# imironhead/ml_super_resolution

Hardware: AMD Instinct MI355X
Metric: VDSR-20 training patches/sec (41x41, batch 256 per GPU); fwd HR megapixels/sec alongside (higher is better)
Workload: dtype f32; 1 GPU; BASELINE configs[2]: VDSR 20-layer 3x3x64 residual, RGB, batch 256x41x41 per GPU, fwd+bwd+TF-Adam, random-init weights; global_batch=256, patch=41, parallelism=dp1

## Files before the change

include/srx.h:

```cpp
#ifndef SRX_H_
#define SRX_H_

#include <stddef.h>
#include <stdint.h>

#ifdef __cplusplus
extern "C" {
#endif

typedef void* srx_stream_t;

typedef enum {
    SRX_OK = 0,
    SRX_ERR_BAD_ARG = -1,
    SRX_ERR_UNSUPPORTED = -2,
    SRX_ERR_WORKSPACE = -3,
    SRX_ERR_LAUNCH = -4,
    SRX_ERR_ALIGN = -5
} srx_status;

typedef enum { SRX_PAD_SAME = 0, SRX_PAD_VALID = 1 } srx_pad_mode;

typedef enum {
    SRX_ACT_NONE = 0,
    SRX_ACT_RELU = 1,
    SRX_ACT_TANH = 2,
    SRX_ACT_LRELU = 3,
    SRX_ACT_SIGMOID = 4
} srx_act;

typedef enum { SRX_OP_FWD = 0, SRX_OP_BWD_DATA = 1, SRX_OP_BWD_FILTER = 2 } srx_conv_op;

typedef enum { SRX_PRECISION_FP32 = 0, SRX_PRECISION_BF16X3 = 1 } srx_precision;

typedef struct {
    int32_t N, H, W, Cin, Cout, KH, KW;
    int32_t stride;
    int32_t pad_mode;
    int32_t act;
    int32_t post_add_relu;
    int32_t precision;
    int32_t subpixel_r;
} srx_conv_desc;

const char* srx_version(void);
const char* srx_last_error(void);

int srx_set_conv_path(int pipelined);

int srx_set_wgrad_path(int path);

int srx_conv_chain(const srx_conv_desc* d, int op, int in_act, int layers, const float* const* x, const float* const* w,
                   const float* const* bias, const float* const* aux, float* const* y, srx_stream_t stream);

int srx_conv_chain_supported(const srx_conv_desc* d, int op, int in_act);

int srx_set_chain(int on);

int srx_conv2d_precision_supported(const srx_conv_desc* d, int op);

size_t srx_conv2d_workspace_bytes(const srx_conv_desc* d, int op);

int srx_conv2d_fwd(const srx_conv_desc* d, const float* x, const float* w, const float* bias,
                   const float* skip, float* y, void* ws, size_t ws_bytes, srx_stream_t stream);

int srx_conv2d_bwd_data(const srx_conv_desc* d, const float* dpre, const float* w,
                        const float* x_in, int in_act, float* dx_out, void* ws, size_t ws_bytes,
                        srx_stream_t stream);

int srx_conv2d_bwd_data_acc(const srx_conv_desc* d, const float* dpre, const float* w, const float* dx_acc,
                            float* dx_out, void* ws, size_t ws_bytes, srx_stream_t stream);

int srx_conv2d_bwd_filter(const srx_conv_desc* d, const float* x, const float* dpre, float* dw,
                          float* dbias, const float* w_for_decay, float wd_scale, void* ws,
                          size_t ws_bytes, srx_stream_t stream);

int srx_conv2d_bwd_filter_partials(const srx_conv_desc* d, const float* x, const float* dpre, void* ws,
                                   size_t ws_bytes, int* n_partials, srx_stream_t stream);
int srx_conv2d_bwd_filter_reduce(const srx_conv_desc* d, const void* ws, int n_partials, float* dw,
                                 float* dbias, const float* w_for_decay, float wd_scale,
                                 srx_stream_t stream);

int srx_act_bwd(const float* dy, const float* y, float* dpre, size_t numel, int act,
                srx_stream_t stream);

int srx_depth_to_space(const float* in, float* out, int N, int H, int W, int C, int r,
                       srx_stream_t stream);

int srx_stream_copy(const void* in, void* out, size_t bytes, srx_stream_t stream);

// ... 145 lines not shown
```

ml_super_resolution_amd/_lib.py:

```python
import ctypes
import os

_HERE = os.path.dirname(os.path.abspath(__file__))
LIB_PATH = os.path.join(_HERE, 'libsrx.so')

SRX_OK = 0
PAD_SAME, PAD_VALID = 0, 1
ACT_NONE, ACT_RELU, ACT_TANH, ACT_LRELU, ACT_SIGMOID = 0, 1, 2, 3, 4
OP_FWD, OP_BWD_DATA, OP_BWD_FILTER = 0, 1, 2
PRECISION_FP32, PRECISION_BF16X3 = 0, 1
PRECISION_BY_NAME = {'highest': PRECISION_FP32, 'high': PRECISION_BF16X3}

ACT_BY_NAME = {None: ACT_NONE, 'none': ACT_NONE, 'relu': ACT_RELU, 'tanh': ACT_TANH,
               'lrelu': ACT_LRELU, 'leaky_relu': ACT_LRELU, 'sigmoid': ACT_SIGMOID}
PAD_BY_NAME = {'same': PAD_SAME, 'valid': PAD_VALID}

EXPORTS = [
    'srx_version', 'srx_last_error', 'srx_set_conv_path', 'srx_set_wgrad_path', 'srx_set_chain', 'srx_conv_chain', 'srx_conv_chain_supported', 'srx_conv2d_precision_supported', 'srx_conv2d_workspace_bytes', 'srx_conv2d_fwd',
    'srx_conv2d_bwd_data', 'srx_conv2d_bwd_filter', 'srx_conv2d_bwd_filter_partials', 'srx_conv2d_bwd_filter_reduce', 'srx_act_bwd', 'srx_depth_to_space',
    'srx_space_to_depth', 'srx_stream_copy', 'srx_mse_fwd_bwd', 'srx_l2_loss', 'srx_reduce_scratch_bytes',
    'srx_adam_tf_step', 'srx_adam_tf_step_dev', 'srx_momentum_clip_step', 'srx_rownorm_loss_fwd_bwd', 'srx_psnr', 'srx_ssim', 'srx_ssim_scratch_bytes', 'srx_saturate_u8', 'srx_affine', 'srx_u8_to_unit_float', 'srx_gaussian_blur', 'srx_resize_bilinear',
    'srx_upsample_nearest', 'srx_upsample_nearest_bwd', 'srx_add_relu_grad',
    'srx_conv2d_bwd_data_acc', 'srx_conv3x3_blocked', 'srx_conv3x3_blocked_bwd_filter_workspace_bytes', 'srx_conv3x3_blocked_bwd_filter',
    'srx_conv3x3_blocked_ex', 'srx_conv3x3_blocked_bwd_filter_ex_workspace_bytes', 'srx_conv3x3_blocked_bwd_filter_ex',
    'srx_espcn_forward', 'srx_espcn_forward_keep', 'srx_debug_poison_lds', 'srx_srcnn_forward', 'srx_maxpool2x2', 'srx_maxpool2x2_bwd', 'srx_maxpool2x2_bwd_masked', 'srx_subsample2', 'srx_subsample2_bwd',
    'srx_channel_blocks_to_nhwc', 'srx_nhwc_to_channel_blocks', 'srx_channel_normalize', 'srx_channel_normalize_bwd',
    'srx_extract_patches16', 'srx_texture_gram', 'srx_texture_gram_bwd', 'srx_pil_resample_ksize', 'srx_pil_resample_coeffs', 'srx_resample_u8', 'srx_u8_to_pm1', 'srx_log_loss', 'srx_vgg_preprocess', 'srx_add_scaled', 'srx_resize_bicubic_tf', 'srx_column_sums', 'srx_gemm_workspace_bytes', 'srx_gemm',
]


class SrxError(RuntimeError):
    pass


class ConvDesc(ctypes.Structure):
    _fields_ = [(n, ctypes.c_int32) for n in
                ('N', 'H', 'W', 'Cin', 'Cout', 'KH', 'KW', 'stride', 'pad_mode', 'act',
                 'post_add_relu', 'precision', 'subpixel_r')]


class GemmDesc(ctypes.Structure):
    _fields_ = ([(n, ctypes.c_int32) for n in ('M', 'N', 'K', 'batch')] +
                [(n, ctypes.c_int64) for n in ('a_row_stride', 'a_col_stride', 'a_batch_stride', 'b_row_stride',
                                               'b_col_stride', 'b_batch_stride', 'c_row_stride', 'c_col_stride',
                                               'c_batch_stride')] +
                [('alpha', ctypes.c_float), ('act', ctypes.c_int32), ('accumulate', ctypes.c_int32)])


_lib = None


def lib():
    global _lib
    if _lib is not None:
        return _lib
    if not os.path.exists(LIB_PATH):
        raise SrxError('libsrx.so not found at %s -- build it with `make -C %s` (or '
                       '__graft_entry__.build()); there is no CPU fallback' %
                       (LIB_PATH, os.path.join(_HERE, 'csrc')))
    import torch
    L = ctypes.CDLL(LIB_PATH)
    vp, sz, i, f = ctypes.c_void_p, ctypes.c_size_t, ctypes.c_int, ctypes.c_float
    dp = ctypes.POINTER(ConvDesc)
    L.srx_version.restype = ctypes.c_char_p
    L.srx_last_error.restype = ctypes.c_char_p
    L.srx_set_conv_path.argtypes = [i]
    L.srx_set_wgrad_path.argtypes = [i]
    L.srx_set_chain.argtypes = [i]
    L.srx_conv_chain_supported.argtypes = [dp, i, i]
    L.srx_conv_chain.argtypes = [dp, i, i, i, vp, vp, vp, vp, vp, vp]
    L.srx_conv2d_precision_supported.argtypes = [dp, i]
    L.srx_conv2d_workspace_bytes.argtypes = [dp, i]
    L.srx_conv2d_workspace_bytes.restype = sz
    L.srx_reduce_scratch_bytes.restype = sz
    L.srx_conv2d_fwd.argtypes = [dp, vp, vp, vp, vp, vp, vp, sz, vp]
    L.srx_conv2d_bwd_data.argtypes = [dp, vp, vp, vp, i, vp, vp, sz, vp]
    L.srx_conv2d_bwd_filter.argtypes = [dp, vp, vp, vp, vp, vp, f, vp, sz, vp]
    L.srx_conv2d_bwd_filter_partials.argtypes = [dp, vp, vp, vp, sz, ctypes.POINTER(ctypes.c_int), vp]
    L.srx_conv2d_bwd_filter_reduce.argtypes = [dp, vp, i, vp, vp, vp, f, vp]
    L.srx_act_bwd.argtypes = [vp, vp, vp, sz, i, vp]
    L.srx_depth_to_space.argtypes = [vp, vp, i, i, i, i, i, vp]
    L.srx_space_to_depth.argtypes = [vp, vp, i, i, i, i, i, vp]
    L.srx_stream_copy.argtypes = [vp, vp, sz, vp]
    L.srx_mse_fwd_bwd.argtypes = [vp, vp, sz, f, vp, i, vp, vp, vp]
    L.srx_l2_loss.argtypes = [vp, vp, sz, f, vp, i, vp, vp]
    L.srx_adam_tf_step.argtypes = [vp, vp, vp, vp, sz, f, f, f, f, ctypes.c_int64, f, vp]
    L.srx_adam_tf_step_dev.argtypes = [vp, vp, vp, vp, sz, vp, f, f, f, f, vp]
    L.srx_momentum_clip_step.argtypes = [vp, vp, vp, sz, f, f, f, f, vp]
    L.srx_rownorm_loss_fwd_bwd.argtypes = [vp, vp, sz, sz, vp, vp, vp, vp]
    L.srx_psnr.argtypes = [vp, vp, vp, i, sz, f, vp]
    L.srx_ssim.argtypes = [vp, vp, vp, i, i, i, i, f, vp, vp]
    L.srx_ssim_scratch_bytes.argtypes = [i]
    L.srx_ssim_scratch_bytes.restype = sz
    L.srx_saturate_u8.argtypes = [vp, vp, sz, vp]
    L.srx_affine.argtypes = [vp, vp, sz, f, f, vp]
    L.srx_u8_to_unit_float.argtypes = [vp, vp, sz, vp]
    L.srx_gaussian_blur.argtypes = [vp, vp, vp, i, i, i, i, f, vp]
    L.srx_resize_bilinear.argtypes = [vp, vp, i, i, i, i, i, i, vp]
    L.srx_upsample_nearest.argtypes = [vp, vp, i, i, i, i, i, vp]
    L.srx_upsample_nearest_bwd.argtypes = [vp, vp, i, i, i, i, i, vp]
    L.srx_add_relu_grad.argtypes = [vp, vp, vp, vp, sz, vp]
# ... 47 lines not shown
```

ml_super_resolution_amd/csrc/conv_narrow.hip:

```cpp
#include "launchers.h"
namespace srx {
typedef float f32x3 __attribute__((ext_vector_type(3)));
typedef unsigned u32x3v __attribute__((ext_vector_type(3)));

template <int CTRL>
__device__ __forceinline__ float dpp_add(float v) {
    const int moved = __builtin_amdgcn_update_dpp(0, __float_as_int(v), CTRL, 0xf, 0xf, false);
    return v + __int_as_float(moved);
}

struct PixWalk {
    int n, oh, ow;
    __device__ __forceinline__ void init(unsigned p, int OH, int OW) {
        const unsigned t = p / (unsigned)OW;
        ow = (int)(p - t * (unsigned)OW);
        n = (int)(t / (unsigned)OH);
        oh = (int)(t - (unsigned)n * (unsigned)OH);
    }
    __device__ __forceinline__ void step16(int OH, int OW) { step(16, OH, OW); }
    __device__ __forceinline__ void step(int d, int OH, int OW) {
        ow += d;
        while (ow >= OW) {
            ow -= OW;
            oh += 1;
            if (oh == OH) { oh = 0; n += 1; }
        }
    }
};
template <int KH, int KW>
__device__ __forceinline__ void tap_offsets(int (&off)[KH * KW], const PixWalk& q, bool live, int H, int W, int pad_t, int pad_l,
                                            int PB, int lane_b) {
    const int centre = ((q.n * H + q.oh - pad_t) * W + (q.ow - pad_l)) * PB + lane_b;
    bool rok[KH], cok[KW];
#pragma unroll
    for (int kh = 0; kh < KH; ++kh) rok[kh] = live && (unsigned)(q.oh + kh - pad_t) < (unsigned)H;
#pragma unroll
    for (int kw = 0; kw < KW; ++kw) cok[kw] = (unsigned)(q.ow + kw - pad_l) < (unsigned)W;
#pragma unroll
    for (int kh = 0; kh < KH; ++kh)
#pragma unroll
        for (int kw = 0; kw < KW; ++kw)
            off[kh * KW + kw] = (rok[kh] && cok[kw]) ? centre + (kh * W + kw) * PB : kOobOffset;
}

template <int KH, int KW, int CIN, int CO>
__global__ __launch_bounds__(256) void conv_narrow_kernel(const ConvArgs a, long total_px, int iters) {
    static_assert(CIN == 64, "16 lanes x 4 channels per pixel");
    constexpr int TAPS = KH * KW;
    const int c4 = threadIdx.x & 15;
    const int sub = threadIdx.x >> 4;
    float wr[TAPS][4][CO];
#pragma unroll
    for (int t = 0; t < TAPS; ++t)
#pragma unroll
        for (int e = 0; e < 4; ++e)
#pragma unroll
            for (int c = 0; c < CO; ++c) wr[t][e][c] = a.w[((size_t)t * CIN + 4 * c4 + e) * CO + c];
    float bias[CO];
#pragma unroll
    for (int c = 0; c < CO; ++c) bias[c] = a.bias ? a.bias[c] : 0.0f;
    const __amdgpu_buffer_rsrc_t xrs = __builtin_amdgcn_make_buffer_rsrc(const_cast<float*>(a.x), 0,
                                                                         a.N * a.H * a.W * CIN * 4, 0x00020000);
    const unsigned p0 = blockIdx.x * (unsigned)iters * 16u + sub;
    PixWalk q;
    q.init(p0 < (unsigned)total_px ? p0 : 0u, a.OH, a.OW);
    for (int it = 0; it < iters; ++it, q.step16(a.OH, a.OW)) {
        const unsigned p = p0 + (unsigned)it * 16u;
        const bool live = p < (unsigned)total_px;
        int off[TAPS];
        tap_offsets<KH, KW>(off, q, live, a.H, a.W, a.pad_t, a.pad_l, CIN * 4, 16 * c4);
        f32x4 v[TAPS];
#pragma unroll
        for (int tp = 0; tp < TAPS; ++tp)
            v[tp] = __builtin_bit_cast(f32x4, __builtin_amdgcn_raw_buffer_load_b128(xrs, off[tp], 0, 0));
        float acc[CO];
#pragma unroll
        for (int c = 0; c < CO; ++c) acc[c] = 0.0f;
// ... 155 lines not shown
```

ml_super_resolution_amd/csrc/launchers.h:

```cpp
#pragma once
#include "conv_kernels.hip.h"

namespace srx {

struct ConvKey {
    int kh, kw, cinp, nch;
    bool wt;
};

bool launch_conv_k3c64(const ConvKey& k, const ConvArgs& a, int grid, size_t lds, hipStream_t s, hipError_t* err);
bool launch_conv_k3c32(const ConvKey& k, const ConvArgs& a, int grid, size_t lds, hipStream_t s, hipError_t* err);
bool launch_conv_c4(const ConvKey& k, const ConvArgs& a, int grid, size_t lds, hipStream_t s, hipError_t* err);
bool launch_conv_misc(const ConvKey& k, const ConvArgs& a, int grid, size_t lds, hipStream_t s, hipError_t* err);
bool launch_pipe_k3c64(const ConvKey& k, const ConvArgs& a, int grid, size_t lds, hipStream_t s, hipError_t* err);
bool launch_pipe_other(const ConvKey& k, const ConvArgs& a, int grid, size_t lds, hipStream_t s, hipError_t* err);
bool launch_wgrad_narrow(const ConvKey& k, const WgradArgs& a, int grid, hipStream_t s, hipError_t* err);
bool launch_conv_narrow(const ConvKey& k, const ConvArgs& a, hipStream_t s, hipError_t* err);
bool launch_conv_1x1(const ConvKey& k, const ConvArgs& a, long min_pixels, hipStream_t s, hipError_t* err);
bool launch_conv_rows3x3(const ConvKey& k, const ConvArgs& a, long min_pixels, hipStream_t s, hipError_t* err);
bool launch_conv_pack3(const ConvKey& k, const ConvArgs& a, long min_pixels, hipStream_t s, hipError_t* err);
bool launch_conv_kwrows(const ConvKey& k, const ConvArgs& a, long min_pixels, hipStream_t s, hipError_t* err);
bool launch_pipe_strip(const ConvKey& k, const ConvArgs& a, int grid, size_t lds, hipStream_t s, hipError_t* err);
bool launch_conv_generic(const ConvKey& k, const ConvArgs& a, int grid, size_t lds, hipStream_t s, hipError_t* err);
bool launch_wgrad(const ConvKey& k, const WgradArgs& a, int grid, size_t lds, hipStream_t s, hipError_t* err);
bool launch_wgrad_generic(const ConvKey& k, const WgradArgs& a, int grid, size_t lds, hipStream_t s, hipError_t* err);
bool launch_wgrad_lin(const ConvKey& k, const WgradArgs& a, int grid, size_t lds, hipStream_t s, hipError_t* err);
bool launch_wgrad_lin_pack3(const ConvKey& k, const WgradArgs& a, int grid, size_t lds, hipStream_t s, hipError_t* err);
bool launch_wgrad_lin_strip(const ConvKey& k, const WgradArgs& a, int grid, size_t lds, hipStream_t s, hipError_t* err);
bool launch_wgrad_pipe(const ConvKey& k, const WgradArgs& a, int grid, size_t lds, hipStream_t s, hipError_t* err);
bool launch_wgrad_kwcols(const ConvKey& k, const WgradArgs& a, int max_partials, long min_pixels, int* n_partials, hipStream_t s, hipError_t* err);
bool launch_wgrad_1x1(const ConvKey& k, const WgradArgs& a, int max_partials, int* n_partials, hipStream_t s, hipError_t* err);
bool launch_wgrad_rows_full(const ConvKey& k, const WgradArgs& a, int grid, size_t lds, hipStream_t s, hipError_t* err);
bool launch_wgrad_rows_strip(const ConvKey& k, const WgradArgs& a, int grid, size_t lds, hipStream_t s, hipError_t* err);
bool launch_wgrad_lin_pairs(const ConvKey& k, const WgradPairs& q, int grid, int pairs, bool strips, size_t lds, hipStream_t s, hipError_t* err);

__attribute__((weak)) hipError_t launch_conv_chain(bool wt, bool aux, const ConvArgs& a, const ChainPtrs& c, int grid, size_t lds, hipStream_t s);

hipError_t launch_reduce_partials(const float* part, int G, int stride, int wn, int cout, float* dw, float* dbias,
                                  const float* w, float wd, hipStream_t s);
hipError_t launch_reduce_partials_pairs(const float* part, int G, int stride, int wn, int cout, float* dw, float* dbias,
                                        int pairs, int cob, hipStream_t s);

template <typename K, typename A>
inline hipError_t launch_with_lds(K kernel, const A& a, int grid, size_t lds, hipStream_t s, int grid_y = 1) {
    static thread_local const void* configured[64];
    static thread_local int n_configured = 0;
    const void* fn = reinterpret_cast<const void*>(kernel);
    bool known = false;
    for (int i = 0; i < n_configured; ++i) known |= (configured[i] == fn);
    if (!known) {
        hipError_t e = hipFuncSetAttribute(fn, hipFuncAttributeMaxDynamicSharedMemorySize, 160 * 1024);
        if (e != hipSuccess) return e;
        if (n_configured < 64) configured[n_configured++] = fn;
    }
    hipLaunchKernelGGL(kernel, dim3(grid, grid_y), dim3(256), lds, s, a);
    return hipGetLastError();
}

template <typename K>
inline hipError_t launch_chain_with_lds(K kernel, const ConvArgs& a, const ChainPtrs& c, int grid, size_t lds, hipStream_t s) {
    static thread_local const void* configured[8];
    static thread_local int n_configured = 0;
    const void* fn = reinterpret_cast<const void*>(kernel);
    bool known = false;
    for (int i = 0; i < n_configured; ++i) known |= (configured[i] == fn);
    if (!known) {
        hipError_t e = hipFuncSetAttribute(fn, hipFuncAttributeMaxDynamicSharedMemorySize, 160 * 1024);
        if (e != hipSuccess) return e;
        if (n_configured < 8) configured[n_configured++] = fn;
// ... 80 lines not shown
```

ml_super_resolution_amd/csrc/srx_api.hip:

```cpp
#include <math.h>
#include <stdarg.h>
#include <atomic>
#include <stdio.h>
#include <stdlib.h>
#include <string.h>

#include "../../include/srx.h"
#include "elementwise.h"
#include "launchers.h"
#include "bf16x3.h"

using namespace srx;

namespace {

thread_local char g_err[512] = "";

struct Knobs {
    int pipe_default, narrow, wgrad_lin, wgrad_pipe, wgrad_pipe_strip, wgrad_rows_full, wgrad_1x1, wgrad_pack3, kwrows_min_pixels, big_route_min_pixels, strip_d2s, conv_1x1_min_pixels, pack3_dgrad;
    int chain;
    unsigned long long* trace;
    int dbg;
};
int env_int(const char* name, int dflt) { const char* e = getenv(name); return e ? atoi(e) : dflt; }
Knobs read_knobs() {
    Knobs k;
    k.pipe_default = env_int("SRX_PIPE", 1);
    k.narrow = env_int("SRX_NARROW", 1);
    k.wgrad_lin = env_int("SRX_WGRAD_LIN", 1);
    k.wgrad_pipe = env_int("SRX_WGRAD_PIPE", 1);
    k.wgrad_pipe_strip = env_int("SRX_WGRAD_PIPE_STRIP", 1);
    k.kwrows_min_pixels = env_int("SRX_KWROWS_MIN_PIXELS", 4096);
    k.big_route_min_pixels = env_int("SRX_BIG_ROUTE_MIN_PIXELS", 60000);
    k.conv_1x1_min_pixels = env_int("SRX_CONV_1X1_MIN_PIXELS", 100000);
    k.pack3_dgrad = env_int("SRX_PACK3_DGRAD", 1);
    k.strip_d2s = env_int("SRX_STRIP_D2S", 1);
    k.wgrad_rows_full = env_int("SRX_WGRAD_ROWS_FULL", 1);
    k.wgrad_1x1 = env_int("SRX_WGRAD_1X1", 1);
    k.wgrad_pack3 = env_int("SRX_WGRAD_PACK3", 1);
    k.chain = env_int("SRX_CHAIN", 1);
    k.trace = nullptr;
    k.dbg = 0;
#ifdef SRX_TRACE
    { const char* tp = getenv("SRX_TRACE_PTR"); k.trace = tp ? (unsigned long long*)strtoull(tp, nullptr, 0) : nullptr; }
    k.dbg = env_int("SRX_DBG", 0);
#endif
    return k;
}
const Knobs& knobs() { static const Knobs k = read_knobs(); return k; }

std::atomic<int> g_use_pipe{-1};
std::atomic<int> g_chain{-1};
int use_chain() { const int v = g_chain.load(std::memory_order_relaxed); return v < 0 ? (knobs().chain ? 1 : 0) : v; }
int use_pipe() { const int v = g_use_pipe.load(std::memory_order_relaxed); return v < 0 ? knobs().pipe_default : v; }
std::atomic<int> g_wgrad_path{-1};
int wgrad_path_default() { return !knobs().wgrad_lin ? 0 : ((knobs().wgrad_pipe || knobs().wgrad_pipe_strip) ? 2 : 1); }
int wgrad_path() { const int v = g_wgrad_path.load(std::memory_order_relaxed); return v < 0 ? wgrad_path_default() : v; }

int cu_count() {
    static std::atomic<int> cached[64];
    int dev = 0;
    if (hipGetDevice(&dev) != hipSuccess || dev < 0 || dev >= 64) { (void)hipGetLastError(); return 256; }
    int n = cached[dev].load(std::memory_order_relaxed);
    if (n > 0) return n;
    if (hipDeviceGetAttribute(&n, hipDeviceAttributeMultiprocessorCount, dev) != hipSuccess || n <= 0) {
        (void)hipGetLastError();
        n = 256;
    }
    if (n > 256) n = 256;
    cached[dev].store(n, std::memory_order_relaxed);
    return n;
}

int fail(int code, const char* fmt, ...) {
    va_list ap;
    va_start(ap, fmt);
    vsnprintf(g_err, sizeof(g_err), fmt, ap);
    va_end(ap);
    return code;
}
}
namespace srx {
int set_error(int code, const char* fmt, ...) {
    va_list ap;
    va_start(ap, fmt);
    vsnprintf(g_err, sizeof(g_err), fmt, ap);
// ... 185 lines not shown
    for (int TW : cands) {
        if (TW > W || TW < 1) continue;
        const long RS = TW + 2;
        long fit = wgrad ? (max_slots - 1 - 2 * RS) / (RS + TW) : max_slots / RS - 2;
        if (fit > H) fit = H;
        for (long th = fit; th >= 1; --th) {
            const long ntx = (W + TW - 1) / TW, nty = (H + th - 1) / th, tiles = (long)N * ntx * nty;
            const long px = th * TW, slots = (th + 2) * RS + (wgrad ? 1 + px : 0), step = wgrad ? 32 : 16;
            const double per_tile = 20.0 * slots + 54.0 * ((px + step - 1) / step * step);
            const long grid = tiles < max_grid ? tiles : max_grid;
            const double cost = (double)((tiles + grid - 1) / grid) * per_tile + 1e-3 * (double)tiles * per_tile / grid;
            if (cost < best) {
                best = cost;
                p->TH = (int)th; p->TW = TW; p->ntx = (int)ntx; p->nty = (int)nty; p->tiles = (int)tiles; p->grid = (int)grid;
                p->lds = (size_t)slots * (wgrad ? kBf3WgradSlot : kBf3ConvSlot);
            }
        }
    }
    if (wgrad && p->lds < 256 * 16) p->lds = 256 * 16;
}

size_t part_stride(const srx_conv_desc* d) {
    const size_t per = (size_t)d->KH * d->KW * d->Cin * d->Cout + (size_t)d->Cout;
    return (per + 3) / 4 * 4;
}

int dispatch_conv(const Plan& p, bool wt, const ConvArgs& a_in, hipStream_t s) {
    ConvKey k{p.KH, p.KW, p.cinp, p.nch, wt};
    hipError_t err = hipSuccess;
    ConvArgs a = a_in;
    const int g_use_pipe = use_pipe();
    const int kPipeGrid = pipe_grid();
    {
        if (knobs().narrow && !a.d2s_r && a.stride == 1 && launch_conv_narrow(k, a, s, &err)) {
            if (err != hipSuccess) return fail(SRX_ERR_LAUNCH, "conv launch failed: %s", hipGetErrorString(err));
            return SRX_OK;
        }
    }
    if (g_use_pipe && knobs().kwrows_min_pixels >= 0 &&
        (launch_conv_kwrows(k, a, knobs().kwrows_min_pixels, s, &err) ||
         ((!k.wt || knobs().pack3_dgrad) &&
          launch_conv_pack3(k, a, k.kh == 9 ? knobs().kwrows_min_pixels : knobs().big_route_min_pixels, s, &err)))) {
        if (err != hipSuccess) return fail(SRX_ERR_LAUNCH, "conv launch failed: %s", hipGetErrorString(err));
        return SRX_OK;
    }
    if (g_use_pipe && knobs().conv_1x1_min_pixels >= 0 && launch_conv_1x1(k, a, knobs().conv_1x1_min_pixels, s, &err)) {
        if (err != hipSuccess) return fail(SRX_ERR_LAUNCH, "conv launch failed: %s", hipGetErrorString(err));
        return SRX_OK;
    }
    const int ppp = 256 / (p.cinp / 4), npart = 4 / p.nch;
    const bool epi_ok = (a.act == ACT_NONE || a.act == ACT_RELU) && (a.post_relu == 0 || a.post_relu == ACT_RELU) && !(a.mask && a.skip) && !(wt && a.skip) && !(!wt && a.mask) &&
                        (!a.mask || (a.mask_act == ACT_RELU && a.act == ACT_NONE && !a.post_relu));
    const bool pipe_ok = epi_ok && !a.d2s_r && a.stride == 1 && a.Cin == p.cinp && p.NTX == 1 && p.RS >= ppp && p.RS == a.W + a.pad_l &&
                         16 * npart <= a.OW && (a.Cout & 3) == 0 &&
                         (long)a.H * a.W * a.Cin * 4 < (1L << 31) - 64 && (long)a.OH * a.OW * a.Cout * 4 < (1L << 31) - 64;
    const bool strip2 = npart == 2 && !wt && !a.skip && !a.mask && !a.post_relu && a.Cout == 32 && p.cinp == 64 &&
                        (a.act == ACT_NONE || a.act == ACT_RELU || a.act == ACT_TANH);
    const bool strip_d2s = knobs().strip_d2s && npart == 2 && !wt && !a.skip && !a.mask && !a.post_relu && a.d2s_r > 0 && a.act == ACT_NONE &&
                           p.cinp == 32 && a.Cout > 16 && a.Cout <= 32 && k.kh == 3 && k.kw == 3 &&
                           (long)a.OH * a.d2s_r * a.OW * a.d2s_r * 3 * 4 < (1L << 31) - 64;
    const bool strip_ok = (epi_ok || strip2 || strip_d2s) && (!a.d2s_r || strip_d2s) && a.stride == 1 && a.Cin == p.cinp && p.NTX > 1 &&
                          (p.TW == 16 || p.TW == 32) && a.OW >= p.TW &&
                          p.RS >= ppp && (npart == 1 || strip2 || strip_d2s) && ((a.Cout & 3) == 0 || strip_d2s) &&
                          a.y != a.skip && a.y != a.mask &&
                          (long)a.H * a.W * a.Cin * 4 < (1L << 31) - 64 && (long)a.OH * a.OW * a.Cout * 4 < (1L << 31) - 64;
    if (g_use_pipe && p.cinp >= 16 && strip_ok) {
        const int pgrid = p.grid < kPipeGrid ? p.grid : kPipeGrid;
// ... 60 lines not shown
    if (op == SRX_OP_FWD && d->act != SRX_ACT_NONE && d->act != SRX_ACT_RELU)
        return fail(SRX_ERR_UNSUPPORTED, "chain: forward activation %d (none / ReLU)", d->act);
    if (op == SRX_OP_BWD_DATA && in_act != SRX_ACT_NONE && in_act != SRX_ACT_RELU)
        return fail(SRX_ERR_UNSUPPORTED, "chain: in_act %d (none / ReLU)", in_act);
    int pt, pl, OH, OW;
    geometry(d, &pt, &pl, &OH, &OW);
    rc = (op == SRX_OP_FWD) ? make_plan(d->N, d->H, d->W, OH, OW, d->Cin, d->Cout, 3, 3, pt, pl, p, true)
                            : make_plan(d->N, OH, OW, d->H, d->W, d->Cout, d->Cin, 3, 3, 2 - pt, 2 - pl, p);
    if (rc) return rc;
    memset(a, 0, sizeof(*a));
    if (op == SRX_OP_FWD) fill_conv_args(a, *p, d->N, d->H, d->W, d->Cin, d->Cout);
    else fill_conv_args(a, *p, d->N, OH, OW, d->Cout, d->Cin);
    a->act = (op == SRX_OP_FWD) ? d->act : SRX_ACT_NONE;
    a->post_relu = 0;
    a->mask_act = (op == SRX_OP_FWD) ? 0 : in_act;
    a->trace = nullptr;
    const int ppp = 256 / (p->cinp / 4);
    const bool pipe_ok = p->cinp == 64 && p->nch == 4 && p->NTX == 1 && p->RS >= ppp && p->RS == a->W + a->pad_l && 16 <= a->OW &&
                         (long)a->H * a->W * a->Cin * 4 < (1L << 31) - 64 && (long)a->OH * a->OW * a->Cout * 4 < (1L << 31) - 64;
    if (!pipe_ok) return fail(SRX_ERR_UNSUPPORTED, "chain: the shape is not on the full-width pipelined route (column strips?)");
    *grid = p->grid < pipe_grid() ? p->grid : pipe_grid();
    if (d->N % *grid) return fail(SRX_ERR_UNSUPPORTED, "chain: N %d is not a multiple of the grid %d (a workgroup would split an image)", d->N, *grid);
    a->buf_floats = (int)(p->lds_bytes / 4);
    return SRX_OK;
}

}

extern "C" {

int srx_set_chain(int on) {
    const int old = g_chain.exchange(on < 0 ? -1 : (on ? 1 : 0), std::memory_order_relaxed);
    return old < 0 ? (knobs().chain ? 1 : 0) : old;
}

int srx_conv_chain_supported(const srx_conv_desc* d, int op, int in_act) {
    Plan p;
    ConvArgs a;
    int grid;
    return chain_plan(d, op, in_act, &p, &a, &grid) == SRX_OK ? 1 : 0;
}

int srx_conv_chain(const srx_conv_desc* d, int op, int in_act, int layers, const float* const* x, const float* const* w,
                   const float* const* bias, const float* const* aux, float* const* y, srx_stream_t stream) {
    if (layers < 1 || layers > kChainMax) return fail(SRX_ERR_BAD_ARG, "chain: %d layers (1..%d)", layers, kChainMax);
    if (!x || !w || !y) return fail(SRX_ERR_BAD_ARG, "null pointer array");
    Plan p;
    ConvArgs a;
    int grid;
    int rc = chain_plan(d, op, in_act, &p, &a, &grid);
    if (rc) return rc;
    const bool wt = op == SRX_OP_BWD_DATA;
    const bool masked = wt && in_act == SRX_ACT_RELU;
    ChainPtrs c;
    memset(&c, 0, sizeof(c));
    c.L = layers;
    for (int l = 0; l < layers; ++l) {
        const float* m = aux ? aux[l] : nullptr;
        if (!x[l] || !w[l] || !y[l]) return fail(SRX_ERR_BAD_ARG, "chain: null tensor pointer in layer %d", l);
        if (!wt && m) return fail(SRX_ERR_UNSUPPORTED, "chain: the forward skip operand is not implemented");
        if (masked != (m != nullptr)) return fail(SRX_ERR_BAD_ARG, "chain: layer %d: a mask goes with in_act ReLU, and only with it", l);
        if (!aligned16(x[l]) || !aligned16(w[l]) || !aligned16(y[l]) || (m && !aligned16(m)) || (bias && bias[l] && (reinterpret_cast<uintptr_t>(bias[l]) & 3)))
            return fail(SRX_ERR_ALIGN, "tensor base pointers must be 16-byte aligned");
        if (y[l] == x[l] || (m && y[l] == m)) return fail(SRX_ERR_BAD_ARG, "chain: layer %d writes its own operand", l);
        c.x[l] = x[l]; c.w[l] = w[l]; c.bias[l] = (bias && !wt) ? bias[l] : nullptr; c.aux[l] = m; c.y[l] = y[l];
    }
// ... 198 lines not shown
    }
    if (!wdone && knobs().big_route_min_pixels >= 0 && wpath >= 1 && !s2) {
        int n1 = 0;
        if (launch_wgrad_kwcols(k, a, p.grid, knobs().big_route_min_pixels, &n1, s, &err)) { wdone = true; wgrid = n1; }
    }
    if (!wdone && use_wpipe && knobs().wgrad_rows_full && lin_ok && d->KH == 3 && d->KW == 3 && d->Cin == 64 && d->Cout == 64 && OW == 41 && d->W == 41 &&
        pl == 1 && pt == 1 && p.RS == 42) {
        WgradArgs ap = a;
        ap.TH = 3;
        ap.zero_slot = (3 + 3) * 42 + 2;
        wgrid = p.grid < kPipeGrid ? p.grid : kPipeGrid;
        wdone = launch_wgrad_rows_full(k, ap, wgrid, 2 * (size_t)(ap.zero_slot + 4) * (64 + 4) * 4, s, &err);
        if (!wdone) wgrid = p.grid;
    }
    if (!wdone && use_wpipe && lin_ok && d->Cin == p.cinp && p.RS >= wppp && 2 * lin_lds <= 160 * 1024) {
        const int kWin = 14 * 4;
        int best_th = 0;
        double best_waste = 1e9;
        for (int th = p.TH; th >= 1; --th) {
            const long pos = (long)th * p.RS, padded = (pos + kWin - 1) / kWin * kWin;
            const double waste = (double)(padded - pos) / (double)pos;
            const bool fits = padded + 2L * p.RS + 6 <= (long)a.zero_slot + 4;
            if (fits && waste < best_waste - 1e-9) { best_waste = waste; best_th = th; }
        }
        if (best_th > 0 && best_waste <= 0.10) {
            WgradArgs ap = a;
            ap.TH = best_th;
            wgrid = p.grid < kPipeGrid ? p.grid : kPipeGrid;
            wdone = launch_wgrad_pipe(k, ap, wgrid, 2 * lin_lds, s, &err);
            if (!wdone) wgrid = p.grid;
        }
    }
    {
        if (!wdone && knobs().narrow && !s2) wdone = launch_wgrad_narrow(k, a, p.grid, s, &err);
    }
    const bool lin_strip_ok = use_lin && p.NTX > 1 && d->Cin == p.cinp && p.RS >= wppp && p.TW >= 4 && lin_lds <= 80 * 1024 &&
                              (OW % p.TW == 0 || OW % p.TW >= 4) && p.RS <= 3 * wppp &&
                              (long)d->H * d->W * d->Cin * 4 < (1L << 31) - 4096 && (long)OH * OW * d->Cout * 4 < (1L << 30);
    const bool rows_ok = wpath >= 2 && knobs().wgrad_pipe_strip && !s2 && p.NTX > 1 && p.TW == 32 && p.RS == 32 + d->KW - 1 &&
                         d->Cin == p.cinp && 2 * lin_lds <= 160 * 1024 &&
                         (long)d->H * d->W * d->Cin * 4 < (1L << 31) - 4096 && (long)OH * OW * d->Cout * 4 < (1L << 30);
    if (!wdone && rows_ok) {
        wgrid = p.grid < kPipeGrid ? p.grid : kPipeGrid;
        wdone = launch_wgrad_rows_strip(k, a, wgrid, 2 * lin_lds, s, &err);
        if (!wdone) wgrid = p.grid;
    }
    if (!wdone && knobs().wgrad_pack3 && lin_ok && lin_lds <= 80 * 1024 && d->Cin == 3) wdone = launch_wgrad_lin_pack3(k, a, p.grid, lin_lds, s, &err);
    if (wdone) {
    } else if (lin_strip_ok && launch_wgrad_lin_strip(k, a, p.grid, lin_lds, s, &err)) {
    } else if (lin_ok && lin_lds <= 80 * 1024 && launch_wgrad_lin(k, a, p.grid, lin_lds, s, &err)) {
    } else if (!launch_wgrad(k, a, p.grid, wg_lds, s, &err) && !(wg_lds <= 80 * 1024 && launch_wgrad_generic(k, a, p.grid, wg_lds, s, &err)))
        return fail(SRX_ERR_UNSUPPORTED, "no wgrad instance for %dx%d, Cin<=%d, Cout chunks %d%s", d->KH, d->KW, p.cinp,
                    p.nch, s2 ? " at stride 2" : "");
    if (err != hipSuccess) return fail(SRX_ERR_LAUNCH, "wgrad launch failed: %s", hipGetErrorString(err));
    *n_partials = wgrid;
    return SRX_OK;
}

int srx_conv2d_bwd_filter_reduce(const srx_conv_desc* d, const void* ws, int n_partials, float* dw, float* dbias,
                                 const float* w_for_decay, float wd_scale, srx_stream_t stream) {
    int rc = check_desc(d);
    if (rc) return rc;
    if (!ws || !dw) return fail(SRX_ERR_BAD_ARG, "null tensor pointer");
    if (d->precision == SRX_PRECISION_BF16X3 && (rc = bf16x3_supported(d, SRX_OP_BWD_FILTER)) != SRX_OK) return rc;
    if (n_partials <= 0 || n_partials > kMaxGridLimit) return fail(SRX_ERR_BAD_ARG, "bad partial count %d", n_partials);
    const size_t wn = (size_t)d->KH * d->KW * d->Cin * d->Cout;
    hipError_t err = launch_reduce_partials((const float*)ws, n_partials, (int)part_stride(d), (int)wn, d->Cout, dw, dbias,
// ... 343 lines not shown
```

ml_super_resolution_amd/ops.py:

```python
import ctypes
import os

import torch

from . import _lib
from ._lib import ACT_BY_NAME, PAD_BY_NAME, ConvDesc, check
from ._lib import lib as _load_lib

_POISON_LDS = os.environ.get('SRX_POISON_LDS', '0') == '1'


def lib():
    L = _load_lib()
    if _POISON_LDS and torch.cuda.is_available():
        L.srx_debug_poison_lds(_stream())
    return L



def _stream():
    return ctypes.c_void_p(torch.cuda.current_stream().cuda_stream)


def _ptr(t):
# ... 90 lines not shown
    return (ctypes.c_void_p * len(ts))(*[None if t is None else t.data_ptr() for t in ts])


def conv2d_fwd_chain(xs, ws, biases, outs, padding='same', act=None):
    for l in range(len(xs)):
        _chk(xs[l], 'x'); _chk(ws[l], 'w'); _chk(biases[l], 'bias'); _chk(outs[l], 'out')
    d = conv_desc(xs[0].shape, ws[0].shape, padding, act)
    shape = out_shape(d)
    for l in range(len(xs)):
        if tuple(xs[l].shape) != tuple(xs[0].shape) or tuple(ws[l].shape) != tuple(ws[0].shape) or tuple(outs[l].shape) != shape:
            raise ValueError('conv2d_fwd_chain: layer %d does not have the shape of layer 0' % l)
    check(lib().srx_conv_chain(ctypes.byref(d), _lib.OP_FWD, _lib.ACT_NONE, len(xs), _ptr_array(xs), _ptr_array(ws), _ptr_array(biases),
                               None, _ptr_array(outs), _stream()), 'srx_conv_chain')
    return outs[-1]


def conv2d_bwd_data_chain(dpres, ws, x_ins, outs, x_shape, padding='same', in_act=None):
    masks = x_ins if (x_ins is not None and in_act is not None) else None
    for l in range(len(dpres)):
        _chk(dpres[l], 'dpre'); _chk(ws[l], 'w'); _chk(outs[l], 'out')
        if masks is not None:
            _chk(masks[l], 'x_in')
        if tuple(outs[l].shape) != tuple(x_shape) or tuple(ws[l].shape) != tuple(ws[0].shape) or tuple(dpres[l].shape) != tuple(dpres[0].shape):
            raise ValueError('conv2d_bwd_data_chain: layer %d does not have the shape of layer 0' % l)
    d = conv_desc(x_shape, ws[0].shape, padding)
    check(lib().srx_conv_chain(ctypes.byref(d), _lib.OP_BWD_DATA, ACT_BY_NAME[in_act] if masks is not None else _lib.ACT_NONE, len(dpres),
                               _ptr_array(dpres), _ptr_array(ws), None, None if masks is None else _ptr_array(masks),
                               _ptr_array(outs), _stream()), 'srx_conv_chain')
    return outs[-1]


def set_chain(on):
    return lib().srx_set_chain(int(on))


def bwd_filter_workspace_bytes(x_shape, w_shape, padding='same', stride=1, precision='highest'):
    d = conv_desc(x_shape, w_shape, padding, stride=stride, precision=precision)
    return lib().srx_conv2d_workspace_bytes(ctypes.byref(d), _lib.OP_BWD_FILTER)


def conv2d_bwd_filter(x, dpre, w_shape, padding='same', w_for_decay=None, wd_scale=0.0, dw=None, dbias=None,
                      want_dbias=True, workspace=None, stride=1, precision='highest'):
    for t, n in ((x, 'x'), (dpre, 'dpre'), (w_for_decay, 'w_for_decay')):
        _chk(t, n)
    d = conv_desc(x.shape, w_shape, padding, stride=stride, precision=precision)
    if tuple(dpre.shape) != tuple(out_shape(d)):
        raise ValueError('dpre has shape %s, the layer output is %s' % (tuple(dpre.shape), tuple(out_shape(d))))
    if dw is None:
        dw = torch.empty(tuple(w_shape), dtype=torch.float32, device=x.device)
    if dbias is None and want_dbias:
        dbias = torch.empty((w_shape[3],), dtype=torch.float32, device=x.device)
    need = lib().srx_conv2d_workspace_bytes(ctypes.byref(d), _lib.OP_BWD_FILTER)
    if workspace is None:
        workspace = torch.empty((need + 3) // 4, dtype=torch.float32, device=x.device)
    check(lib().srx_conv2d_bwd_filter(ctypes.byref(d), _ptr(x), _ptr(dpre), _ptr(dw), _ptr(dbias),
                                      _ptr(w_for_decay), float(wd_scale), _ptr(workspace),
                                      workspace.numel() * 4, _stream()), 'srx_conv2d_bwd_filter')
    return dw, dbias


def conv2d_bwd_filter_partials(x, dpre, w_shape, padding, workspace, precision='highest'):
    _chk(x, 'x'); _chk(dpre, 'dpre'); _chk(workspace, 'workspace')
    d = conv_desc(x.shape, w_shape, padding, precision=precision)
    n = ctypes.c_int(0)
    check(lib().srx_conv2d_bwd_filter_partials(ctypes.byref(d), _ptr(x), _ptr(dpre), _ptr(workspace), workspace.numel() * 4,
                                               ctypes.byref(n), _stream()), 'srx_conv2d_bwd_filter_partials')
# ... 534 lines not shown
```

Before: 18930 patches/s.

## Add LDS ring-buffer tiled kernels for 64->3 narrow conv and wgrad

Adds new kernels for the 3x3 64-to-3 output layer, both forward conv and weight gradient. Each block streams consecutive pixel chunks through a shared-memory ring buffer, so every input pixel is loaded from global memory once and its nine taps are served from LDS instead of being read again per tap. The new path is on by default through an env knob and falls back to the old narrow kernels when its shape conditions fail. The cost is more LDS per block, a barrier on every iteration and more complex addressing, and it affects only one layer of the network.

```diff
diff --git a/include/srx.h b/include/srx.h
--- a/include/srx.h
+++ b/include/srx.h
@@ -56,6 +56,8 @@
 int srx_conv_chain_supported(const srx_conv_desc* d, int op, int in_act);
 
 int srx_set_chain(int on);
+
+int srx_set_narrow_tiled(int on);
 
 int srx_conv2d_precision_supported(const srx_conv_desc* d, int op);
 
diff --git a/ml_super_resolution_amd/_lib.py b/ml_super_resolution_amd/_lib.py
--- a/ml_super_resolution_amd/_lib.py
+++ b/ml_super_resolution_amd/_lib.py
@@ -16,7 +16,7 @@
 PAD_BY_NAME = {'same': PAD_SAME, 'valid': PAD_VALID}
 
 EXPORTS = [
-    'srx_version', 'srx_last_error', 'srx_set_conv_path', 'srx_set_wgrad_path', 'srx_set_chain', 'srx_conv_chain', 'srx_conv_chain_supported', 'srx_conv2d_precision_supported', 'srx_conv2d_workspace_bytes', 'srx_conv2d_fwd',
+    'srx_version', 'srx_last_error', 'srx_set_conv_path', 'srx_set_wgrad_path', 'srx_set_chain', 'srx_set_narrow_tiled', 'srx_conv_chain', 'srx_conv_chain_supported', 'srx_conv2d_precision_supported', 'srx_conv2d_workspace_bytes', 'srx_conv2d_fwd',
     'srx_conv2d_bwd_data', 'srx_conv2d_bwd_filter', 'srx_conv2d_bwd_filter_partials', 'srx_conv2d_bwd_filter_reduce', 'srx_act_bwd', 'srx_depth_to_space',
     'srx_space_to_depth', 'srx_stream_copy', 'srx_mse_fwd_bwd', 'srx_l2_loss', 'srx_reduce_scratch_bytes',
     'srx_adam_tf_step', 'srx_adam_tf_step_dev', 'srx_momentum_clip_step', 'srx_rownorm_loss_fwd_bwd', 'srx_psnr', 'srx_ssim', 'srx_ssim_scratch_bytes', 'srx_saturate_u8', 'srx_affine', 'srx_u8_to_unit_float', 'srx_gaussian_blur', 'srx_resize_bilinear',
@@ -67,6 +67,7 @@
     L.srx_set_conv_path.argtypes = [i]
     L.srx_set_wgrad_path.argtypes = [i]
     L.srx_set_chain.argtypes = [i]
+    L.srx_set_narrow_tiled.argtypes = [i]
     L.srx_conv_chain_supported.argtypes = [dp, i, i]
     L.srx_conv_chain.argtypes = [dp, i, i, i, vp, vp, vp, vp, vp, vp]
     L.srx_conv2d_precision_supported.argtypes = [dp, i]
diff --git a/ml_super_resolution_amd/csrc/conv_narrow.h b/ml_super_resolution_amd/csrc/conv_narrow.h
--- /dev/null
+++ b/ml_super_resolution_amd/csrc/conv_narrow.h
@@ -0,0 +1,46 @@
+#pragma once
+#include "launchers.h"
+namespace srx {
+typedef float f32x3 __attribute__((ext_vector_type(3)));
+typedef unsigned u32x3v __attribute__((ext_vector_type(3)));
+
+template <int CTRL>
+__device__ __forceinline__ float dpp_add(float v) {
+    const int moved = __builtin_amdgcn_update_dpp(0, __float_as_int(v), CTRL, 0xf, 0xf, false);
+    return v + __int_as_float(moved);
+}
+
+struct PixWalk {
+    int n, oh, ow;
+    __device__ __forceinline__ void init(unsigned p, int OH, int OW) {
+        const unsigned t = p / (unsigned)OW;
+        ow = (int)(p - t * (unsigned)OW);
+        n = (int)(t / (unsigned)OH);
+        oh = (int)(t - (unsigned)n * (unsigned)OH);
+    }
+    __device__ __forceinline__ void step16(int OH, int OW) { step(16, OH, OW); }
+    __device__ __forceinline__ void step(int d, int OH, int OW) {
+        ow += d;
+        while (ow >= OW) {
+            ow -= OW;
+            oh += 1;
+            if (oh == OH) { oh = 0; n += 1; }
+        }
+    }
+};
+template <int KH, int KW>
+__device__ __forceinline__ void tap_offsets(int (&off)[KH * KW], const PixWalk& q, bool live, int H, int W, int pad_t, int pad_l,
+                                            int PB, int lane_b) {
+    const int centre = ((q.n * H + q.oh - pad_t) * W + (q.ow - pad_l)) * PB + lane_b;
+    bool rok[KH], cok[KW];
+#pragma unroll
+    for (int kh = 0; kh < KH; ++kh) rok[kh] = live && (unsigned)(q.oh + kh - pad_t) < (unsigned)H;
+#pragma unroll
+    for (int kw = 0; kw < KW; ++kw) cok[kw] = (unsigned)(q.ow + kw - pad_l) < (unsigned)W;
+#pragma unroll
+    for (int kh = 0; kh < KH; ++kh)
+#pragma unroll
+        for (int kw = 0; kw < KW; ++kw)
+            off[kh * KW + kw] = (rok[kh] && cok[kw]) ? centre + (kh * W + kw) * PB : kOobOffset;
+}
+}
diff --git a/ml_super_resolution_amd/csrc/conv_narrow.hip b/ml_super_resolution_amd/csrc/conv_narrow.hip
--- a/ml_super_resolution_amd/csrc/conv_narrow.hip
+++ b/ml_super_resolution_amd/csrc/conv_narrow.hip
@@ -1,48 +1,5 @@
-#include "launchers.h"
+#include "conv_narrow.h"
 namespace srx {
-typedef float f32x3 __attribute__((ext_vector_type(3)));
-typedef unsigned u32x3v __attribute__((ext_vector_type(3)));
-
-template <int CTRL>
-__device__ __forceinline__ float dpp_add(float v) {
-    const int moved = __builtin_amdgcn_update_dpp(0, __float_as_int(v), CTRL, 0xf, 0xf, false);
-    return v + __int_as_float(moved);
-}
-
-struct PixWalk {
-    int n, oh, ow;
-    __device__ __forceinline__ void init(unsigned p, int OH, int OW) {
-        const unsigned t = p / (unsigned)OW;
-        ow = (int)(p - t * (unsigned)OW);
-        n = (int)(t / (unsigned)OH);
-        oh = (int)(t - (unsigned)n * (unsigned)OH);
-    }
-    __device__ __forceinline__ void step16(int OH, int OW) { step(16, OH, OW); }
-    __device__ __forceinline__ void step(int d, int OH, int OW) {
-        ow += d;
-        while (ow >= OW) {
-            ow -= OW;
-            oh += 1;
-            if (oh == OH) { oh = 0; n += 1; }
-        }
-    }
-};
-template <int KH, int KW>
-__device__ __forceinline__ void tap_offsets(int (&off)[KH * KW], const PixWalk& q, bool live, int H, int W, int pad_t, int pad_l,
-                                            int PB, int lane_b) {
-    const int centre = ((q.n * H + q.oh - pad_t) * W + (q.ow - pad_l)) * PB + lane_b;
-    bool rok[KH], cok[KW];
-#pragma unroll
-    for (int kh = 0; kh < KH; ++kh) rok[kh] = live && (unsigned)(q.oh + kh - pad_t) < (unsigned)H;
-#pragma unroll
-    for (int kw = 0; kw < KW; ++kw) cok[kw] = (unsigned)(q.ow + kw - pad_l) < (unsigned)W;
-#pragma unroll
-    for (int kh = 0; kh < KH; ++kh)
-#pragma unroll
-        for (int kw = 0; kw < KW; ++kw)
-            off[kh * KW + kw] = (rok[kh] && cok[kw]) ? centre + (kh * W + kw) * PB : kOobOffset;
-}
-
 template <int KH, int KW, int CIN, int CO>
 __global__ __launch_bounds__(256) void conv_narrow_kernel(const ConvArgs a, long total_px, int iters) {
     static_assert(CIN == 64, "16 lanes x 4 channels per pixel");
diff --git a/ml_super_resolution_amd/csrc/conv_narrow_tiled.hip b/ml_super_resolution_amd/csrc/conv_narrow_tiled.hip
--- /dev/null
+++ b/ml_super_resolution_amd/csrc/conv_narrow_tiled.hip
@@ -0,0 +1,248 @@
+#include "conv_narrow.h"
+namespace srx {
+namespace {
+constexpr int kSlotB = 256;
+constexpr int kChunkB = 16 * kSlotB;
+constexpr int kDQ = 4;
+
+struct RingStage {
+    __amdgpu_buffer_rsrc_t rs;
+    char* ring;
+    int total, lane_b, sub, mask_b, k_last;
+    __device__ __forceinline__ f32x4 load(int k) const {
+        const int px = 16 * k + sub;
+        const bool ok = px >= 0 && px < total && k <= k_last;
+        return __builtin_bit_cast(f32x4, __builtin_amdgcn_raw_buffer_load_b128(rs, ok ? px * kSlotB + lane_b : kOobOffset, 0, 0));
+    }
+    __device__ __forceinline__ void store(int k, const f32x4 v) const {
+        *reinterpret_cast<f32x4*>(ring + (((16 * k + sub) * kSlotB + lane_b) & mask_b)) = v;
+    }
+};
+
+template <typename F>
+__device__ __forceinline__ void ring_walk(const RingStage& st, int c0, int iters, int A, F&& body) {
+    if (threadIdx.x < kSlotB / 4) reinterpret_cast<float*>(st.ring + st.mask_b + 1)[threadIdx.x] = 0.0f;
+    for (int k = c0 - A; k < c0 + A; k += kDQ) {
+        f32x4 v[kDQ];
+#pragma unroll
+        for (int j = 0; j < kDQ; ++j) v[j] = st.load(k + j);
+#pragma unroll
+        for (int j = 0; j < kDQ; ++j)
+            if (k + j < c0 + A) st.store(k + j, v[j]);
+    }
+    f32x4 q[kDQ];
+#pragma unroll
+    for (int j = 0; j < kDQ; ++j) q[j] = st.load(c0 + A + j);
+    for (int it0 = 0; it0 < iters; it0 += kDQ) {
+#pragma unroll
+        for (int j = 0; j < kDQ; ++j) {
+            const int it = it0 + j;
+            if (it < iters) {
+                st.store(c0 + it + A, q[j]);
+                q[j] = st.load(c0 + it + A + kDQ);
+                __syncthreads();
+                body(it);
+            }
+        }
+    }
+}
+
+__device__ __forceinline__ void tap_slots(int (&ad)[9], const PixWalk& q, unsigned p, bool live, int H, int W, int pad_t, int pad_l,
+                                          int lane_b, int mask_b) {
+    const int base = ((int)p - pad_t * W - pad_l) * kSlotB + lane_b;
+    const int zero = mask_b + 1 + lane_b;
+    bool rok[3], cok[3];
+#pragma unroll
+    for (int kh = 0; kh < 3; ++kh) rok[kh] = live && (unsigned)(q.oh + kh - pad_t) < (unsigned)H;
+#pragma unroll
+    for (int kw = 0; kw < 3; ++kw) cok[kw] = (unsigned)(q.ow + kw - pad_l) < (unsigned)W;
+#pragma unroll
+    for (int kh = 0; kh < 3; ++kh)
+#pragma unroll
+        for (int kw = 0; kw < 3; ++kw)
+            ad[kh * 3 + kw] = (rok[kh] && cok[kw]) ? ((base + (kh * W + kw) * kSlotB) & mask_b) : zero;
+}
+}
+
+__global__ __launch_bounds__(256) void conv_narrow_tiled_kernel(const ConvArgs a, int total_px, int iters, int A, int mask_b) {
+    constexpr int TAPS = 9, CIN = 64, CO = 3;
+    extern __shared__ __attribute__((aligned(16))) char ring[];
+    const int c4 = threadIdx.x & 15;
+    const int sub = threadIdx.x >> 4;
+    float wr[TAPS][4][CO];
+#pragma unroll
+    for (int t = 0; t < TAPS; ++t)
+#pragma unroll
+        for (int e = 0; e < 4; ++e)
+#pragma unroll
+            for (int c = 0; c < CO; ++c) wr[t][e][c] = a.w[((size_t)t * CIN + 4 * c4 + e) * CO + c];
+    float bias[CO];
+#pragma unroll
+    for (int c = 0; c < CO; ++c) bias[c] = a.bias ? a.bias[c] : 0.0f;
+    const int c0 = blockIdx.x * iters;
+    RingStage st;
+    st.rs = __builtin_amdgcn_make_buffer_rsrc(const_cast<float*>(a.x), 0, a.N * a.H * a.W * CIN * 4, 0x00020000);
+    st.ring = ring; st.total = total_px; st.lane_b = 16 * c4; st.sub = sub; st.mask_b = mask_b; st.k_last = c0 + iters - 1 + A;
+    const unsigned p0 = (unsigned)c0 * 16u + sub;
+    PixWalk q;
+    q.init(p0 < (unsigned)total_px ? p0 : 0u, a.OH, a.OW);
+    ring_walk(st, c0, iters, A, [&](int it) __attribute__((always_inline)) {
+        const unsigned p = p0 + (unsigned)it * 16u;
+        const bool live = p < (unsigned)total_px;
+        int ad[TAPS];
+        tap_slots(ad, q, p, live, a.H, a.W, a.pad_t, a.pad_l, 16 * c4, mask_b);
+        f32x4 v[TAPS];
+#pragma unroll
+        for (int tp = 0; tp < TAPS; ++tp) v[tp] = *reinterpret_cast<const f32x4*>(ring + ad[tp]);
+        float acc[CO];
+#pragma unroll
+        for (int c = 0; c < CO; ++c) acc[c] = 0.0f;
+#pragma unroll
+        for (int tp = 0; tp < TAPS; ++tp)
+#pragma unroll
+            for (int e = 0; e < 4; ++e)
+#pragma unroll
+                for (int c = 0; c < CO; ++c) acc[c] = fmaf(v[tp][e], wr[tp][e][c], acc[c]);
+#pragma unroll
+        for (int c = 0; c < CO; ++c) {
+            float r = acc[c];
+            r = dpp_add<0xB1>(r);
+            r = dpp_add<0x4E>(r);
+            r = dpp_add<0x124>(r);
+            r = dpp_add<0x128>(r);
+            acc[c] = r;
+        }
+        if (live && c4 < CO) {
+            float r = (c4 == 0) ? acc[0] : (c4 == 1 ? acc[1] : acc[2]);
+            r = act_apply(r + ((c4 == 0) ? bias[0] : (c4 == 1 ? bias[1] : bias[2])), a.act);
+            const size_t o = (size_t)p * CO + c4;
+            if (a.skip) r += a.skip[o];
+            if (a.post_relu) r = act_apply(r, a.post_relu);
+            a.y[o] = r;
+        }
+        q.step16(a.OH, a.OW);
+    });
+}
+
+__global__ __launch_bounds__(256) void wgrad_narrow_tiled_kernel(const WgradArgs a, int total_px, int iters, int A, int mask_b) {
+    constexpr int TAPS = 9, CN = 3, CW = 64, LPP = 16;
+    constexpr int NV = TAPS * 4 * CN + CN;
+    extern __shared__ __attribute__((aligned(16))) char ring[];
+    float* red = reinterpret_cast<float*>(ring);
+    const int c4 = threadIdx.x & (LPP - 1);
+    const int sub = threadIdx.x / LPP;
+    const int wave = threadIdx.x >> 6;
+    float acc[NV];
+#pragma unroll
+    for (int i = 0; i < NV; ++i) acc[i] = 0.0f;
+    const __amdgpu_buffer_rsrc_t drs = __builtin_amdgcn_make_buffer_rsrc(
+        const_cast<float*>(a.dpre), 0, a.N * a.OH * a.OW * CN * 4, 0x00020000);
+    const int c0 = blockIdx.x * iters;
+    RingStage st;
+    st.rs = __builtin_amdgcn_make_buffer_rsrc(const_cast<float*>(a.x), 0, a.N * a.H * a.W * CW * 4, 0x00020000);
+    st.ring = ring; st.total = total_px; st.lane_b = 16 * c4; st.sub = sub; st.mask_b = mask_b; st.k_last = c0 + iters - 1 + A;
+    const unsigned p0 = (unsigned)c0 * 16u + sub;
+    PixWalk q;
+    q.init(p0 < (unsigned)total_px ? p0 : 0u, a.OH, a.OW);
+    ring_walk(st, c0, iters, A, [&](int it) __attribute__((always_inline)) {
+        const unsigned p = p0 + (unsigned)it * 16u;
+        const bool live = p < (unsigned)total_px;
+        int ad[TAPS];
+        tap_slots(ad, q, p, live, a.H, a.W, a.pad_t, a.pad_l, 16 * c4, mask_b);
+        const f32x3 d = __builtin_bit_cast(f32x3, __builtin_amdgcn_raw_buffer_load_b96(drs, live ? (int)(p * CN * 4) : kOobOffset, 0, 0));
+        f32x4 v[TAPS];
+#pragma unroll
+        for (int tp = 0; tp < TAPS; ++tp) v[tp] = *reinterpret_cast<const f32x4*>(ring + ad[tp]);
+#pragma unroll
+        for (int tp = 0; tp < TAPS; ++tp)
+#pragma unroll
+            for (int e = 0; e < 4; ++e)
+#pragma unroll
+                for (int c = 0; c < CN; ++c) acc[(tp * 4 + e) * CN + c] = fmaf(v[tp][e], d[c], acc[(tp * 4 + e) * CN + c]);
+#pragma unroll
+        for (int c = 0; c < CN; ++c) acc[TAPS * 4 * CN + c] += d[c];
+        q.step16(a.OH, a.OW);
+    });
+    __syncthreads();
+#pragma unroll
+    for (int i = 0; i < NV; ++i) {
+        float r = acc[i];
+#pragma unroll
+        for (int o = LPP; o < 64; o <<= 1) r += __shfl_xor(r, o);
+        if (sub % (64 / LPP) == 0) red[(wave * NV + i) * LPP + c4] = r;
+    }
+    __syncthreads();
+    float* part = a.part + (size_t)blockIdx.x * a.part_stride;
+    const int wn = TAPS * CW * CN;
+    for (int j = threadIdx.x; j < NV * LPP; j += 256) {
+        const int i = j / LPP, l = j % LPP;
+        const float r = (red[(0 * NV + i) * LPP + l] + red[(1 * NV + i) * LPP + l]) +
+                        (red[(2 * NV + i) * LPP + l] + red[(3 * NV + i) * LPP + l]);
+        if (i < TAPS * 4 * CN) {
+            const int c = i % CN, te = i / CN, e = te & 3, tp = te >> 2;
+            part[(tp * CW + 4 * l + e) * CN + c] = r;
+        } else if (l == 0) {
+            part[wn + i - TAPS * 4 * CN] = r;
+        }
+    }
+}
+
+namespace {
+bool ring_plan(int W, int pad_t, int pad_l, int* A, int* mask_b, size_t* lds) {
+    if (pad_t < 0 || pad_t > 2 || pad_l < 0 || pad_l > 2) return false;
+    const int back = pad_t * W + pad_l, ahead = (2 - pad_t) * W + (2 - pad_l);
+    const int ab = (back + 15) / 16, af = (15 + ahead) / 16;
+    *A = ab > af ? ab : af;
+    int rc = 8;
+    while (rc < 2 * *A + 2) rc *= 2;
+    if (rc > 16) return false;
+    *mask_b = rc * kChunkB - 1;
+    *lds = (size_t)rc * kChunkB + kSlotB;
+    return true;
+}
+template <typename K>
+hipError_t ring_launch(K kernel, size_t lds) {
+    static thread_local const void* configured[2];
+    const void* fn = reinterpret_cast<const void*>(kernel);
+    if (lds <= 64 * 1024 || configured[0] == fn || configured[1] == fn) return hipSuccess;
+    const hipError_t e = hipFuncSetAttribute(fn, hipFuncAttributeMaxDynamicSharedMemorySize, 16 * kChunkB + kSlotB);
+    if (e == hipSuccess) configured[configured[0] ? 1 : 0] = fn;
+    return e;
+}
+}
+
+bool launch_conv_narrow_tiled(const ConvKey& k, const ConvArgs& a, int grid, hipStream_t s, hipError_t* err) {
+    if (k.wt || k.kh != 3 || k.kw != 3 || a.Cin != 64 || a.Cout != 3 || a.mask || a.stride != 1 || a.OH != a.H || a.OW != a.W) return false;
+    const long total = (long)a.N * a.OH * a.OW;
+    if (total * 64 * 4 >= (1L << 31) - 4096) return false;
+    int A, mask_b;
+    size_t lds;
+    if (!ring_plan(a.W, a.pad_t, a.pad_l, &A, &mask_b, &lds)) return false;
+    const long chunks = (total + 15) / 16;
+    int iters = (int)((chunks + grid - 1) / grid);
+    if (iters < 8) iters = 8;
+    const long blocks = (chunks + iters - 1) / iters;
+    if ((blocks * iters + A + kDQ + 1) * kChunkB >= (1L << 31)) return false;
+    if ((*err = ring_launch(conv_narrow_tiled_kernel, lds)) != hipSuccess) return true;
+    hipLaunchKernelGGL(conv_narrow_tiled_kernel, dim3((unsigned)blocks), dim3(256), lds, s, a, (int)total, iters, A, mask_b);
+    *err = hipGetLastError();
+    return true;
+}
+
+bool launch_wgrad_narrow_tiled(const ConvKey& k, const WgradArgs& a, int grid, hipStream_t s, hipError_t* err) {
+    if (k.kh != 3 || k.kw != 3 || a.Cin != 64 || a.Cout != 3 || a.stride != 1 || a.OH != a.H || a.OW != a.W) return false;
+    const long total = (long)a.N * a.OH * a.OW;
+    if (total * 64 * 4 >= (1L << 31) - 4096) return false;
+    int A, mask_b;
+    size_t lds;
+    if (!ring_plan(a.W, a.pad_t, a.pad_l, &A, &mask_b, &lds)) return false;
+    const size_t red = 4 * (size_t)(9 * 4 * 3 + 3) * 16 * sizeof(float);
+    if (lds < red) lds = red;
+    const int iters = (int)((total + 16L * grid - 1) / (16L * grid));
+    if (((long)grid * iters + A + kDQ + 1) * kChunkB >= (1L << 31)) return false;
+    if ((*err = ring_launch(wgrad_narrow_tiled_kernel, lds)) != hipSuccess) return true;
+    hipLaunchKernelGGL(wgrad_narrow_tiled_kernel, dim3(grid), dim3(256), lds, s, a, (int)total, iters, A, mask_b);
+    *err = hipGetLastError();
+    return true;
+}
+}
diff --git a/ml_super_resolution_amd/csrc/launchers.h b/ml_super_resolution_amd/csrc/launchers.h
--- a/ml_super_resolution_amd/csrc/launchers.h
+++ b/ml_super_resolution_amd/csrc/launchers.h
@@ -35,6 +35,9 @@
 bool launch_wgrad_lin_pairs(const ConvKey& k, const WgradPairs& q, int grid, int pairs, bool strips, size_t lds, hipStream_t s, hipError_t* err);
 
 __attribute__((weak)) hipError_t launch_conv_chain(bool wt, bool aux, const ConvArgs& a, const ChainPtrs& c, int grid, size_t lds, hipStream_t s);
+
+__attribute__((weak)) bool launch_conv_narrow_tiled(const ConvKey& k, const ConvArgs& a, int grid, hipStream_t s, hipError_t* err);
+__attribute__((weak)) bool launch_wgrad_narrow_tiled(const ConvKey& k, const WgradArgs& a, int grid, hipStream_t s, hipError_t* err);
 
 hipError_t launch_reduce_partials(const float* part, int G, int stride, int wn, int cout, float* dw, float* dbias,
                                   const float* w, float wd, hipStream_t s);
diff --git a/ml_super_resolution_amd/csrc/srx_api.hip b/ml_super_resolution_amd/csrc/srx_api.hip
--- a/ml_super_resolution_amd/csrc/srx_api.hip
+++ b/ml_super_resolution_amd/csrc/srx_api.hip
@@ -18,7 +18,7 @@
 
 struct Knobs {
     int pipe_default, narrow, wgrad_lin, wgrad_pipe, wgrad_pipe_strip, wgrad_rows_full, wgrad_1x1, wgrad_pack3, kwrows_min_pixels, big_route_min_pixels, strip_d2s, conv_1x1_min_pixels, pack3_dgrad;
-    int chain;
+    int chain, narrow_tiled;
     unsigned long long* trace;
     int dbg;
 };
@@ -39,6 +39,7 @@
     k.wgrad_1x1 = env_int("SRX_WGRAD_1X1", 1);
     k.wgrad_pack3 = env_int("SRX_WGRAD_PACK3", 1);
     k.chain = env_int("SRX_CHAIN", 1);
+    k.narrow_tiled = env_int("SRX_NARROW_TILED", 1);
     k.trace = nullptr;
     k.dbg = 0;
 #ifdef SRX_TRACE
@@ -52,6 +53,8 @@
 std::atomic<int> g_use_pipe{-1};
 std::atomic<int> g_chain{-1};
 int use_chain() { const int v = g_chain.load(std::memory_order_relaxed); return v < 0 ? (knobs().chain ? 1 : 0) : v; }
+std::atomic<int> g_narrow_tiled{-1};
+int use_narrow_tiled() { const int v = g_narrow_tiled.load(std::memory_order_relaxed); return v < 0 ? (knobs().narrow_tiled ? 1 : 0) : v; }
 int use_pipe() { const int v = g_use_pipe.load(std::memory_order_relaxed); return v < 0 ? knobs().pipe_default : v; }
 std::atomic<int> g_wgrad_path{-1};
 int wgrad_path_default() { return !knobs().wgrad_lin ? 0 : ((knobs().wgrad_pipe || knobs().wgrad_pipe_strip) ? 2 : 1); }
@@ -303,7 +306,8 @@
     const int g_use_pipe = use_pipe();
     const int kPipeGrid = pipe_grid();
     {
-        if (knobs().narrow && !a.d2s_r && a.stride == 1 && launch_conv_narrow(k, a, s, &err)) {
+        if (knobs().narrow && !a.d2s_r && a.stride == 1 &&
+            ((use_narrow_tiled() && launch_conv_narrow_tiled && launch_conv_narrow_tiled(k, a, max_grid(), s, &err)) || launch_conv_narrow(k, a, s, &err))) {
             if (err != hipSuccess) return fail(SRX_ERR_LAUNCH, "conv launch failed: %s", hipGetErrorString(err));
             return SRX_OK;
         }
@@ -430,6 +434,11 @@
 int srx_set_chain(int on) {
     const int old = g_chain.exchange(on < 0 ? -1 : (on ? 1 : 0), std::memory_order_relaxed);
     return old < 0 ? (knobs().chain ? 1 : 0) : old;
+}
+
+int srx_set_narrow_tiled(int on) {
+    const int old = g_narrow_tiled.exchange(on < 0 ? -1 : (on ? 1 : 0), std::memory_order_relaxed);
+    return old < 0 ? (knobs().narrow_tiled ? 1 : 0) : old;
 }
 
 int srx_conv_chain_supported(const srx_conv_desc* d, int op, int in_act) {
@@ -694,7 +703,8 @@
         }
     }
     {
-        if (!wdone && knobs().narrow && !s2) wdone = launch_wgrad_narrow(k, a, p.grid, s, &err);
+        if (!wdone && knobs().narrow && !s2)
+            wdone = (use_narrow_tiled() && launch_wgrad_narrow_tiled && launch_wgrad_narrow_tiled(k, a, p.grid, s, &err)) || launch_wgrad_narrow(k, a, p.grid, s, &err);
     }
     const bool lin_strip_ok = use_lin && p.NTX > 1 && d->Cin == p.cinp && p.RS >= wppp && p.TW >= 4 && lin_lds <= 80 * 1024 &&
                               (OW % p.TW == 0 || OW % p.TW >= 4) && p.RS <= 3 * wppp &&
diff --git a/ml_super_resolution_amd/ops.py b/ml_super_resolution_amd/ops.py
--- a/ml_super_resolution_amd/ops.py
+++ b/ml_super_resolution_amd/ops.py
@@ -146,6 +146,10 @@
 
 def set_chain(on):
     return lib().srx_set_chain(int(on))
+
+
+def set_narrow_tiled(on):
+    return lib().srx_set_narrow_tiled(int(on))
 
 
 def bwd_filter_workspace_bytes(x_shape, w_shape, padding='same', stride=1, precision='highest'):
```

New measurement: 18920 patches/s. No clear change (-0.0%).
